# cheshmi/parsy_bench

Measured on AMD Instinct MI355X. Metric: Cholesky factorizations/sec (+ SpTRSV solves/sec), SuiteSparse SPD set, higher is better.
Workload: dtype f64; 1 GPU; flan-class stand-in (BASELINE.json configs[2] when flan: Flan_1565): grid (116, 116, 116) 27-point stencil, geometric nested dissection; n=1560896, nnz_A_lower=21491316, nsuper=81191, nnz_L=2044454227, xsize=2421483055, etree_levels=17, launches_per_factorization=357, parallelism=1 GPU

## Files before the change

### include/parsy_amd.h

```cpp
#ifndef PARSY_AMD_H
#define PARSY_AMD_H

#include <stdbool.h>
#include <stddef.h>
#include <stdint.h>

#ifdef __cplusplus
extern "C" {
#endif


bool cholesky_left_par_05(int n, int* c, int* r, double* values, size_t* lC, int* lR,
                          size_t* Li_ptr, double* lValues, int* blockSet, int supNo,
                          double* timing, int* aTree, int* cT, int* rT, int* col2Sup,
                          int nLevels, int* levelPtr, int* levelSet, int nPar, int* parPtr,
                          int* partition, int chunk, int threads, int super_max, int col_max,
                          double* nodCost);

bool cholesky_left_par_05_prune(int n, int* c, int* r, double* values, size_t* lC, int* lR,
                                size_t* Li_ptr, double* lValues, int* blockSet, int supNo,
                                double* timing, int* prunePtr, int* pruneSet, int nLevels,
                                int* levelPtr, int* levelSet, int nPar, int* parPtr, int* partition,
                                int chunk, int threads, int super_max, int col_max, double* nodCost);

// ... 52 lines not shown
    int32_t solve_one;
    int32_t solve_one_blocks;
    int32_t sub_mrhs_trees;
    int32_t sub_mrhs_slots;
    int32_t sub_mrhs_tiers;
    int32_t sub_mrhs_cover_level;
    int64_t dense_strip_entries;
} parsy_plan_info;

parsy_plan* parsy_plan_create(int n, int supNo, const int* blockSet, const size_t* lC,
                              const size_t* Li_ptr, const int* lR, const int* aTree,
                              const int* col2Sup, const int* cT, const int* rT, const int* c,
                              const int* r, int device);
void parsy_plan_destroy(parsy_plan* plan);
int parsy_plan_get_info(const parsy_plan* plan, parsy_plan_info* info);

int parsy_plan_set_active(parsy_plan* plan, const uint8_t* mask);
long long parsy_plan_chain_check(const parsy_plan* plan, int slots);
long long parsy_plan_check(const parsy_plan* plan);

int parsy_factor_device(parsy_plan* plan, const double* d_values, double* d_lValues,
                        void* stream);
#define PARSY_FACTOR_NO_INIT 1
int parsy_factor_device_ex(parsy_plan* plan, const double* d_values, double* d_lValues,
                           void* stream, int flags);
int parsy_factor_status(parsy_plan* plan);

int parsy_factor_begin(parsy_plan* plan, const double* d_values, double* d_lValues, void* stream, int flags);
int parsy_factor_level(parsy_plan* plan, int level, double* d_lValues, void* stream);
int parsy_factor_end(parsy_plan* plan, void* stream);
int parsy_plan_pieces(const parsy_plan* plan, int32_t* supernode, int32_t* level, int32_t* col0, int32_t* width,
                      int32_t* rows, int64_t* value_begin, int64_t* value_end);
int parsy_plan_set_active_pieces(parsy_plan* plan, const uint8_t* piece_mask);

typedef struct parsy_dist parsy_dist;
typedef struct parsy_dist_info {
    int32_t nranks, nlevels, n_pieces, n_subtrees, n_root_pieces, n_messages;
    int64_t exchange_elements;
    double total_cost, root_cost;
    double max_rank_cost;
    double lockstep_cost;
} parsy_dist_info;
parsy_dist* parsy_dist_create(const parsy_plan* plan, int nranks, int block);
void parsy_dist_destroy(parsy_dist* dist);
int parsy_dist_get_info(const parsy_dist* dist, parsy_dist_info* info);
int parsy_dist_get(const parsy_dist* dist, int32_t* owner, uint8_t* in_subtree, double* rank_cost,
                   double* level_cost);
int parsy_dist_level_messages(const parsy_dist* dist, int level);
int parsy_dist_message(const parsy_dist* dist, int level, int index, int32_t* src, int32_t* dst, int64_t* nseg,
                       int64_t* total, const int64_t** off, const int32_t** len, const int64_t** packed);
long long parsy_dist_check(const parsy_plan* plan, const parsy_dist* dist);

int parsy_solve_device(parsy_plan* plan, const double* d_lValues, double* d_x, int nrhs,
                       int ldx, void* stream);

int parsy_solve_status(parsy_plan* plan);

int parsy_backsolve_device(parsy_plan* plan, const double* d_lValues, double* d_x, int nrhs, int ldx,
                           void* stream);
int parsy_plan_solve_levels(const parsy_plan* plan, int32_t* level);
#define PARSY_SOLVE_FIRST 1
#define PARSY_SOLVE_LAST 2
#define PARSY_SOLVE_BACKWARD 4
int parsy_solve_levels_device(parsy_plan* plan, const double* d_lValues, double* d_x, int nrhs, int ldx, void* stream,
                              int level_begin, int level_end, int flags);
int parsy_rhs_ones_device(parsy_plan* plan, const double* d_lValues, double* d_b, void* stream);
// ... 163 lines not shown
```

### parsy_bench_amd/_native.py

```python
from __future__ import annotations

import ctypes as C
import os
from pathlib import Path

import numpy as np

_PKG = Path(__file__).resolve().parent
_LIB_PATH = Path(os.environ["PARSY_LIB"]) if os.environ.get("PARSY_LIB") else _PKG / "libparsy_amd.so"
_lib = None

c_int_p = C.POINTER(C.c_int)
c_dbl_p = C.POINTER(C.c_double)
c_size_p = C.POINTER(C.c_size_t)
c_i64_p = C.POINTER(C.c_int64)


class SymbolicView(C.Structure):
    _fields_ = [
        ("n", C.c_int32), ("nsuper", C.c_int32), ("nlevels", C.c_int32),
        ("maxSupWid", C.c_int32), ("maxCol", C.c_int32),
        ("ssize", C.c_int64), ("xsize", C.c_int64), ("nnzL", C.c_int64),
        ("nnzA", C.c_int64), ("n_updates", C.c_int64),
        ("flops_colcount", C.c_double), ("flops_stored", C.c_double),
# ... 29 lines not shown
        ("sub_mrhs_tiers", C.c_int32), ("sub_mrhs_cover_level", C.c_int32),
        ("dense_strip_entries", C.c_int64),
    ]

    def as_dict(self):
        return {k: getattr(self, k) for k, _ in self._fields_}


EXPORTED_SYMBOLS = [
    "cholesky_left_par_05", "cholesky_left_par_05_prune", "cholesky_left_par_waveFront", "blockedLsolve",
    "leveledBlockedLsolve", "H2LeveledBlockedLsolve", "H2LeveledBlockedLsolve_Peeled",
    "parsy_dropin_reset", "parsy_plan_create", "parsy_plan_destroy", "parsy_plan_get_info",
    "parsy_plan_set_active", "parsy_plan_chain_check", "parsy_factor_device", "parsy_factor_status", "parsy_solve_device",
    "parsy_factor_host", "parsy_solve_host", "parsy_last_factor_ms", "parsy_last_solve_ms",
    "parsy_last_error", "parsy_device_count", "parsy_analyze", "parsy_symbolic_free",
    "parsy_symbolic_get", "parsy_plan_from_symbolic", "parsy_grid_spd_lower",
    "parsy_grid_nested_dissection", "parsy_order_nd", "parsy_plan_profile", "parsy_plan_profile_collect",
    "parsy_plan_profile_get", "parsy_factor_device_ex", "parsy_backsolve_device", "parsy_solve_levels_device", "parsy_plan_solve_levels", "parsy_solve2_host",
    "parsy_rhs_ones_device", "parsy_solve_status", "parsy_copy_segments_device", "parsy_plan_check",
    "parsy_factor_begin", "parsy_factor_level", "parsy_factor_end", "parsy_plan_pieces",
    "parsy_plan_set_active_pieces", "parsy_dist_create", "parsy_dist_destroy", "parsy_dist_get_info",
    "parsy_dist_get", "parsy_dist_level_messages", "parsy_dist_message", "parsy_dist_check",
    "parsy_mg_create", "parsy_mg_destroy", "parsy_mg_set_values", "parsy_mg_factor", "parsy_mg_rank_ms",
    "parsy_mg_gather_host", "parsy_mg_dist", "parsy_mg_plan", "parsy_mg_profile", "parsy_plan_profile_levels",
    "parsy_debug_kernel_count", "parsy_debug_kernel_name", "parsy_debug_kernel_launches", "parsy_debug_kernel_reset",
    "parsy_plan_set_perm", "parsy_residual_device", "parsy_solve_spd_device", "parsy_solve_spd_host",
    "parsy_selinv_get_info", "parsy_selinv_check", "parsy_selinv_device", "parsy_inverse_diag_device",
    "parsy_selinv_host", "parsy_logdet_device",
    "parsy_plan_pattern", "parsy_grad_get_info", "parsy_pattern_outer_device", "parsy_inverse_pattern_device",
    "parsy_trace_inverse_device", "parsy_pattern_outer_host", "parsy_inverse_pattern_host",
    "parsy_cond_get_info", "parsy_error_bounds_device", "parsy_solve_spd_bounds_device", "parsy_solve_spd_bounds_host",
    "parsy_rcond_device", "parsy_rcond_host",
    "parsy_factor_apply_device", "parsy_factor_apply_host", "parsy_factor_apply_get_info", "parsy_factor_apply_row_index",
]


class ApplyInfo(C.Structure):
    _fields_ = [
        ("rows", C.c_int32), ("max_occurrences", C.c_int32), ("occurrences", C.c_int64), ("block_columns", C.c_int32),
        ("last_op", C.c_int32), ("last_launches", C.c_int32), ("reserved", C.c_int32), ("workspace_bytes", C.c_int64),
        ("device_bytes", C.c_int64),
    ]

    def as_dict(self):
        return {k: getattr(self, k) for k, _ in self._fields_ if k != "reserved"}


class CondInfo(C.Structure):
    _fields_ = [("applications", C.c_int32), ("columns", C.c_int32), ("device_bytes", C.c_int64)]

    def as_dict(self):
        return {k: getattr(self, k) for k, _ in self._fields_}


class GradInfo(C.Structure):
    _fields_ = [
        ("entries", C.c_int64), ("offdiag_entries", C.c_int64), ("device_bytes", C.c_int64), ("last_lanes", C.c_int32),
    ]

    def as_dict(self):
        return {k: getattr(self, k) for k, _ in self._fields_}


class SelinvInfo(C.Structure):
    _fields_ = [
        ("levels", C.c_int32), ("block_columns", C.c_int32), ("tiled_block_columns", C.c_int32),
# ... 31 lines not shown
    lib.parsy_symbolic_free.argtypes = [vp]
    lib.parsy_symbolic_get.argtypes = [vp, C.POINTER(SymbolicView)]
    lib.parsy_grid_spd_lower.restype = C.c_int64
    lib.parsy_grid_spd_lower.argtypes = [C.c_int, C.c_int, C.c_int, C.c_int, C.c_double, vp, vp, vp]
    lib.parsy_grid_nested_dissection.argtypes = [C.c_int, C.c_int, C.c_int, C.c_int, vp]
    lib.parsy_order_nd.argtypes = [C.c_int, vp, vp, C.c_int, vp]
    lib.parsy_plan_create.restype = vp
    lib.parsy_plan_create.argtypes = [C.c_int, C.c_int] + [vp] * 10 + [C.c_int]
    lib.parsy_plan_from_symbolic.restype = vp
    lib.parsy_plan_from_symbolic.argtypes = [vp, C.c_int]
    lib.parsy_plan_destroy.argtypes = [vp]
    lib.parsy_plan_get_info.argtypes = [vp, C.POINTER(PlanInfo)]
    lib.parsy_plan_set_active.argtypes = [vp, vp]
    lib.parsy_plan_chain_check.argtypes = [vp, C.c_int]
    lib.parsy_plan_chain_check.restype = C.c_longlong
    lib.parsy_plan_check.argtypes = [vp]
    lib.parsy_plan_check.restype = C.c_longlong
    lib.parsy_factor_device.argtypes = [vp, vp, vp, vp]
    lib.parsy_factor_device_ex.argtypes = [vp, vp, vp, vp, C.c_int]
    lib.parsy_factor_status.argtypes = [vp]
    lib.parsy_solve_device.argtypes = [vp, vp, vp, C.c_int, C.c_int, vp]
    lib.parsy_plan_solve_levels.argtypes = [vp, vp]
    lib.parsy_solve_levels_device.argtypes = [vp, vp, vp, C.c_int, C.c_int, vp, C.c_int, C.c_int, C.c_int]
    lib.parsy_backsolve_device.argtypes = [vp, vp, vp, C.c_int, C.c_int, vp]
    lib.parsy_solve2_host.argtypes = [vp, vp, vp, C.c_int, C.c_int, C.c_int, vp]
    lib.parsy_rhs_ones_device.argtypes = [vp, vp, vp, vp]
    lib.parsy_solve_status.argtypes = [vp]
    lib.parsy_copy_segments_device.argtypes = [vp, vp, vp, vp, vp, C.c_int64, vp]
    lib.parsy_factor_begin.argtypes = [vp, vp, vp, vp, C.c_int]
    lib.parsy_factor_level.argtypes = [vp, C.c_int, vp, vp]
    lib.parsy_factor_end.argtypes = [vp, vp]
    lib.parsy_plan_pieces.argtypes = [vp] + [vp] * 7
    lib.parsy_plan_set_active_pieces.argtypes = [vp, vp]
    lib.parsy_dist_create.restype = vp
    lib.parsy_dist_create.argtypes = [vp, C.c_int, C.c_int]
    lib.parsy_dist_destroy.argtypes = [vp]
    lib.parsy_dist_get_info.argtypes = [vp, C.POINTER(DistInfo)]
    lib.parsy_dist_get.argtypes = [vp, vp, vp, vp, vp]
    lib.parsy_dist_level_messages.argtypes = [vp, C.c_int]
    lib.parsy_dist_message.argtypes = [vp, C.c_int, C.c_int, c_int_p, c_int_p, c_i64_p, c_i64_p,
                                       C.POINTER(c_i64_p), C.POINTER(c_int_p), C.POINTER(c_i64_p)]
    lib.parsy_dist_check.argtypes = [vp, vp]
    lib.parsy_dist_check.restype = C.c_longlong
    lib.parsy_mg_create.restype = vp
    lib.parsy_mg_create.argtypes = [vp, C.c_int, vp, C.c_int]
    lib.parsy_mg_destroy.argtypes = [vp]
    lib.parsy_mg_set_values.argtypes = [vp, vp]
    lib.parsy_mg_factor.argtypes = [vp, vp]
    lib.parsy_mg_rank_ms.argtypes = [vp, vp]
    lib.parsy_mg_profile.argtypes = [vp, vp, vp, vp]
    lib.parsy_plan_profile_levels.argtypes = [vp, vp, vp]
    lib.parsy_mg_gather_host.argtypes = [vp, vp]
    lib.parsy_mg_dist.restype = vp
    lib.parsy_mg_dist.argtypes = [vp]
    lib.parsy_mg_plan.restype = vp
    lib.parsy_mg_plan.argtypes = [vp, C.c_int]
    lib.parsy_plan_set_perm.argtypes = [vp, vp]
    lib.parsy_residual_device.argtypes = [vp, vp, vp, C.c_int, vp, C.c_int, vp, C.c_int, C.c_int, vp, vp]
    lib.parsy_solve_spd_device.argtypes = [vp, vp, vp, vp, C.c_int, vp, C.c_int, C.c_int, C.c_int, vp, vp, vp]
    lib.parsy_solve_spd_host.argtypes = [vp, vp, vp, vp, C.c_int, vp, C.c_int, C.c_int, C.c_int, vp, vp, vp]
    lib.parsy_cond_get_info.argtypes = [vp, vp]
    lib.parsy_error_bounds_device.argtypes = [vp, vp, vp, vp, C.c_int, vp, C.c_int, C.c_int, vp, vp, vp]
    lib.parsy_solve_spd_bounds_device.argtypes = [vp, vp, vp, vp, C.c_int, vp, C.c_int, C.c_int, C.c_int, vp, vp, vp, vp]
    lib.parsy_solve_spd_bounds_host.argtypes = [vp, vp, vp, vp, C.c_int, vp, C.c_int, C.c_int, C.c_int, vp, vp, vp, vp]
    lib.parsy_rcond_device.argtypes = [vp, vp, vp, vp, vp, vp]
    lib.parsy_rcond_host.argtypes = [vp, vp, vp, vp, vp, vp]
# ... 83 lines not shown
```

### parsy_bench_amd/api.py

```python
from __future__ import annotations

import ctypes as C

import numpy as np

from . import _native as N

KIND_NAMES = ["SMALL", "TILES", "CHAIN", "BIG", "BACK_BELOW", "SOLVE_SMALL", "SOLVE_PANEL", "SOLVE_FIXUP", "BACK_BLOCK", "DENSE"]


def device_count() -> int:
    return int(N.lib().parsy_device_count())


def kernel_launches() -> dict:
    lib = N.lib()
    return {lib.parsy_debug_kernel_name(k).decode(): int(lib.parsy_debug_kernel_launches(k))
            for k in range(lib.parsy_debug_kernel_count())}


def reset_kernel_launches() -> None:
    N.lib().parsy_debug_kernel_reset()


# ... 433 lines not shown
            raise RuntimeError("parsy_solve_device failed: " + N.last_error())

    def solve_levels(self) -> np.ndarray:
        out = np.zeros(self.sym.nsuper, dtype=np.int32)
        N.lib().parsy_plan_solve_levels(self._h, N.ptr(out))
        return out

    def solve_levels_device(self, d_lValues: int, d_x: int, nrhs: int, ldx: int, stream: int, level_begin: int, level_end: int,
                            first: bool, last: bool, backward: bool = False) -> None:
        flags = (1 if first else 0) | (2 if last else 0) | (4 if backward else 0)
        if N.lib().parsy_solve_levels_device(self._h, d_lValues, d_x, nrhs, ldx, stream, level_begin, level_end, flags) != 0:
            raise RuntimeError("parsy_solve_levels_device failed: " + N.last_error())

    def factor_begin(self, d_values: int, d_lValues: int, stream: int = 0, init: bool = True) -> None:
        if N.lib().parsy_factor_begin(self._h, d_values, d_lValues, stream, 0 if init else 1) != 0:
            raise RuntimeError("parsy_factor_begin failed: " + N.last_error())

    def factor_level(self, level: int, d_lValues: int, stream: int = 0) -> None:
        if N.lib().parsy_factor_level(self._h, level, d_lValues, stream) != 0:
            raise RuntimeError("parsy_factor_level failed: " + N.last_error())

    def factor_end(self, stream: int = 0) -> None:
        if N.lib().parsy_factor_end(self._h, stream) != 0:
            raise RuntimeError("parsy_factor_end failed: " + N.last_error())

    def pieces(self) -> dict:
        n = int(N.lib().parsy_plan_pieces(self._h, *([None] * 7)))
        out = {k: np.zeros(n, dtype=np.int32) for k in ("supernode", "level", "col0", "width", "rows")}
        out.update({k: np.zeros(n, dtype=np.int64) for k in ("value_begin", "value_end")})
        N.lib().parsy_plan_pieces(self._h, *[N.ptr(out[k]) for k in (
            "supernode", "level", "col0", "width", "rows", "value_begin", "value_end")])
        return out

    def set_active_pieces(self, mask) -> None:
        m = None if mask is None else np.ascontiguousarray(mask, dtype=np.uint8)
        if N.lib().parsy_plan_set_active_pieces(self._h, N.ptr(m)) != 0:
            raise RuntimeError(N.last_error())

    def check(self) -> int:
        return int(N.lib().parsy_plan_check(self._h))

    def last_factor_ms(self) -> float:
        return float(N.lib().parsy_last_factor_ms(self._h))

    def last_solve_ms(self) -> float:
        return float(N.lib().parsy_last_solve_ms(self._h))

    def profile(self, mode: int) -> None:
        N.lib().parsy_plan_profile(self._h, mode)

    def profile_collect(self) -> None:
        if N.lib().parsy_plan_profile_collect(self._h) != 0:
            raise RuntimeError("profile_collect: no profiled run to collect")

    def profile_get(self) -> dict:
        ms = np.zeros(10, dtype=np.float64)
        cnt = np.zeros(10, dtype=np.int32)
        runs = C.c_int(0)
        N.lib().parsy_plan_profile_get(self._h, N.ptr(ms), N.ptr(cnt), C.byref(runs))
        return {"runs": runs.value, "ms": dict(zip(KIND_NAMES, ms.tolist())),
                "launches": dict(zip(KIND_NAMES, cnt.tolist()))}


class Dist:

    def __init__(self, plan: "Plan", nranks: int, block: int = 0, _borrowed=None):
# ... 106 lines not shown
```

### parsy_bench_amd/csrc/capi_exec.hip

```cpp
#include <hip/hip_runtime.h>

#include <chrono>
#include <cstdio>
#include <cstring>
#include <map>
#include <algorithm>
#include <mutex>
#include <string>
#include <tuple>
#include <vector>

#include "../../include/parsy_amd.h"
#include "errors.hpp"
#include "hip_check.hpp"
#include "dist.hpp"
#include "executor.hpp"
#include "inspector.hpp"
#include "plan_util.hpp"
#include "refine.hpp"
#include "cond.hpp"
#include "apply.hpp"

using parsy::set_last_error;

// ... 348 lines not shown
    parsy::build_launches(pl->S, mask, pl->piece_mask_set ? pieces.data() : nullptr);
    pl->sn_mask_set = mask != nullptr;
    return parsy::plan_upload_launches(pl);
}

int parsy_plan_set_active_pieces(parsy_plan* pl, const uint8_t* piece_mask) {
    if (!pl) return -1;
    std::vector<uint8_t> sn_mask;
    if (pl->sn_mask_set) sn_mask = pl->S.active;
    parsy::build_launches(pl->S, pl->sn_mask_set ? sn_mask.data() : nullptr, piece_mask);
    pl->piece_mask_set = piece_mask != nullptr;
    return parsy::plan_upload_launches(pl);
}

int parsy_plan_pieces(const parsy_plan* pl, int32_t* supernode, int32_t* level, int32_t* col0, int32_t* width,
                      int32_t* rows, int64_t* value_begin, int64_t* value_end) {
    if (!pl) return -1;
    const parsy::Schedule& S = pl->S;
    const int nc = (int)S.csn.size();
    for (int p = 0; p < nc; ++p) {
        const parsy::SnDesc& C = S.csn[(size_t)p];
        const parsy::SnDesc& R = S.sn[(size_t)S.csn_real[(size_t)p]];
        if (supernode) supernode[p] = S.csn_real[(size_t)p];
        if (level) level[p] = S.level_of.empty() ? 0 : S.level_of[(size_t)p];
        if (col0) col0[p] = C.c0;
        if (width) width[p] = C.w;
        if (rows) rows[p] = C.r;
        if (value_begin) value_begin[p] = R.px + (int64_t)C.rbias * R.r;
        if (value_end) value_end[p] = R.px + (int64_t)(C.rbias + C.w) * R.r;
    }
    return nc;
}

int parsy_plan_solve_levels(const parsy_plan* pl, int32_t* level) {
    if (!pl) return -1;
    const parsy::Schedule& S = pl->S;
    if (level)
        for (int l = 0; l < S.nlevels; ++l)
            for (int q = S.levelPtr[(size_t)l]; q < S.levelPtr[(size_t)l + 1]; ++q) level[S.levelSet[(size_t)q]] = l;
    return S.nlevels;
}

int64_t parsy_debug_big_entries(const parsy_plan* pl, int32_t* out, int64_t cap) {
    if (!pl) return -1;
    const parsy::Schedule& S = pl->S;
    int64_t n = 0, t = 0;
    for (const parsy::Schedule::BigTask& b : S.big_all) {
        for (int64_t e = b.e0; e < b.e1; ++e, ++n) {
            if (!out || n >= cap) continue;
            const parsy::WaveEntry& E = S.big_entries[(size_t)e];
            int32_t* o = out + 7 * n;
            o[0] = (int32_t)t;
            o[1] = b.src_level * 2 + (b.next ? 0 : 1);
            o[2] = E.K;
            o[3] = E.mn & 255;
            o[4] = (E.mn >> 8) & 255;
            o[5] = ((E.mn >> 16) & 1) != 0;
            o[6] = E.ia - E.ja;
        }
        ++t;
    }
    return n;
}

int64_t parsy_debug_big_windows(const parsy_plan* pl, int64_t* out, int64_t cap) {
    if (!pl) return -1;
// ... 398 lines not shown
```

### parsy_bench_amd/csrc/executor.hip

```cpp
#include "executor.hpp"

#include <climits>
#include <cstdlib>
#include <cstring>
#include <stdexcept>

#include "apply.hpp"
#include "cond.hpp"
#include "device_util.hpp"
#include "errors.hpp"
#include "grad.hpp"
#include "hip_check.hpp"
#include "plan_fwd.hpp"
#include "plan_util.hpp"
#include "refine.hpp"
#include "selinv.hpp"

namespace parsy {

const Schedule& plan_schedule(const parsy_plan* plan) { return plan->S; }

int check_plan(const parsy_plan* pl, const char* who, PlanNeeds needs) {
    const std::string w(who);
    if (pl->device < 0) return set_last_error(w + ": plan was built without a device (device < 0)"), -1;
// ... 202 lines not shown
        PARSY_HIP(hipMalloc(&d, sbytes));
        pl->owned.push_back(d);
        pl->dp.tile_scratch = (double*)d;
        pl->device_bytes += (int64_t)sbytes;
    }
    {
        void* d = nullptr;
        PARSY_HIP(hipMalloc(&d, sizeof(int)));
        pl->owned.push_back(d);
        pl->dp.info = (int*)d;
        PARSY_HIP(hipMemset(d, 0x7f, sizeof(int)));
        PARSY_HIP(hipMalloc(&d, sizeof(int)));
        pl->owned.push_back(d);
        pl->dp.sinfo = (int*)d;
        PARSY_HIP(hipMemset(d, 0, sizeof(int)));
        const size_t tbytes = 2 * std::max<int64_t>(S.n_tflags, 1) * sizeof(int);
        pl->dp.n_tflags = (int)S.n_tflags;
        PARSY_HIP(hipMalloc(&d, tbytes));
        pl->owned.push_back(d);
        pl->dp.tflags = (int*)d;
        PARSY_HIP(hipMemset(d, 0, tbytes));
        pl->device_bytes += (int64_t)tbytes;
    }
    {
        int prio_least = 0, prio_greatest = 0;
        PARSY_HIP(hipDeviceGetStreamPriorityRange(&prio_least, &prio_greatest));
        PARSY_HIP(hipStreamCreateWithPriority(&pl->side_stream, hipStreamNonBlocking, prio_least));
    }
    PARSY_HIP(hipEventCreateWithFlags(&pl->ev_init, hipEventDisableTiming));
    pl->ev_level_done.resize(std::max(S.nlevels, S.cnlevels) + 1);
    pl->ev_early_done.resize(std::max(S.nlevels, S.cnlevels) + 1);
    for (auto& e : pl->ev_level_done) PARSY_HIP(hipEventCreateWithFlags(&e, hipEventDisableTiming));
    for (auto& e : pl->ev_early_done) PARSY_HIP(hipEventCreateWithFlags(&e, hipEventDisableTiming));
    {
        const char* no = std::getenv("PARSY_NO_OVERLAP");
        pl->overlap = !(no && no[0] == '1');
    }
    PARSY_HIP(hipEventCreate(&pl->ev_f0));
    PARSY_HIP(hipEventCreate(&pl->ev_f1));
    PARSY_HIP(hipEventCreate(&pl->ev_s0));
    PARSY_HIP(hipEventCreate(&pl->ev_s1));
    return plan_upload_launches(pl);
}

parsy_plan* plan_build(const PatternRef& P, const size_t* lC, const int* A2p, const int* A2i,
                       int device) {
    parsy_plan* pl = new parsy_plan;
    int cus = 0;
    if (device >= 0) {
        hipDeviceProp_t prop;
        if (hipGetDeviceProperties(&prop, device) == hipSuccess) cus = prop.multiProcessorCount;
        (void)hipSetDevice(device);
        const int per_cu = chain_workgroups_per_cu();
        if (per_cu == 1) cus = cus / 2;
    }
    try {
        build_schedule(P, lC, A2p, A2i, nullptr, pl->S, cus);
    } catch (const std::exception& e) {
        set_last_error(std::string("plan: ") + e.what());
        delete pl;
        return nullptr;
    }
    pl->solve_only = pl->S.solve_only;
    pl->device = device;
    if (device >= 0 && plan_upload(pl) != 0) {
        plan_free(pl);
        return nullptr;
    }
    return pl;
}

void plan_free(parsy_plan* pl) {
    if (!pl) return;
    if (pl->device >= 0) {
        (void)hipSetDevice(pl->device);
        (void)hipDeviceSynchronize();
        for (void* d : pl->owned) (void)hipFree(d);
        for (void* d : pl->launch_owned) (void)hipFree(d);
        if (pl->xscratch) (void)hipFree(pl->xscratch);
        for (double*& q : pl->one_y) {
            if (q) (void)hipFree(q);
            q = nullptr;
        }
        if (pl->xt) (void)hipFree(pl->xt);
        if (pl->d_perm) (void)hipFree(pl->d_perm);
        if (pl->dinv) (void)hipFree(pl->dinv);
        if (pl->dp.bpart) (void)hipFree(pl->dp.bpart);
        if (pl->h_values_dev) (void)hipFree(pl->h_values_dev);
        if (pl->h_L_dev) (void)hipFree(pl->h_L_dev);
        if (pl->h_x_dev) (void)hipFree(pl->h_x_dev);
        for (hipEvent_t e : {pl->ev_f0, pl->ev_f1, pl->ev_s0, pl->ev_s1})
            if (e) (void)hipEventDestroy(e);
        for (hipEvent_t e : pl->pev) (void)hipEventDestroy(e);
        for (hipEvent_t e : pl->ev_level_done) (void)hipEventDestroy(e);
        for (hipEvent_t e : pl->ev_early_done) (void)hipEventDestroy(e);
        if (pl->ev_init) (void)hipEventDestroy(pl->ev_init);
        if (pl->side_stream) (void)hipStreamDestroy(pl->side_stream);
        if (pl->h_stream) (void)hipStreamDestroy(pl->h_stream);
        if (pl->h_copy) (void)hipStreamDestroy(pl->h_copy);
        for (hipEvent_t e : pl->h_band_ev) (void)hipEventDestroy(e);
    }
    refine_free(pl);
    selinv_free(pl);
    grad_free(pl);
    cond_free(pl);
    apply_free(pl);
    delete pl;
}

static void profile_mark(parsy_plan* pl, int kind, hipStream_t stream, size_t& cursor, int level = -1, int side = 0,
                         int count = 0) {
    if (!pl->profile) return;
    if (cursor >= pl->pev_count.size()) pl->pev_count.resize(cursor + 1, 0);
    pl->pev_count[cursor] = count;
    if (cursor >= pl->pev_level.size()) pl->pev_level.resize(cursor + 1, 0);
    pl->pev_level[cursor] = level >= 0 ? (level << 1) | (side & 1) : -1;
    if (cursor >= pl->pev.size()) {
        hipEvent_t e;
        (void)hipEventCreate(&e);
        pl->pev.push_back(e);
    }
    if (cursor >= pl->pev_kind.size()) pl->pev_kind.push_back(kind);
    else pl->pev_kind[cursor] = kind;
    (void)hipEventRecord(pl->pev[cursor], stream);
    ++cursor;
}

static bool sub_tiers_usable(const parsy_plan* pl, int nrhs, int ldx) {
    const int m = pl->dp.gates.sub_mrhs_min;
    return pl->dp.sub_ntiers > 0 && m > 0 && nrhs >= m && ldx < (1 << 24) && nrhs < (1 << 20);
}

static void run_begin(parsy_plan* pl) {
    pl->run_cursor = 0;
    pl->run_next_level_event = 0;
    pl->run_early_seen.assign(pl->ev_early_done.size(), 0);
}

static void run_range(parsy_plan* pl, const std::vector<Launch>& seq, size_t i0, size_t i1, double* L,
                      const double* Lc, double* x, int nrhs, int ldx, hipStream_t stream) {
    size_t& cursor = pl->run_cursor;
    const bool overlap = pl->overlap && !pl->profile && pl->side_stream != nullptr;
    int& next_level_event = pl->run_next_level_event;
    std::vector<char>& early_seen = pl->run_early_seen;
    auto record_levels_below = [&](int level) {
        for (; next_level_event < level && next_level_event < (int)pl->ev_level_done.size(); ++next_level_event)
            (void)hipEventRecord(pl->ev_level_done[next_level_event], stream);
    };
    for (size_t li = i0; li < i1; ++li) {
        const Launch& l = seq[li];
        const bool on_side = overlap && l.side;
        if (!on_side) {
            if (overlap && is_chol_launch(l.kind)) record_levels_below(l.level);
            if (overlap && (l.kind == kLaunchChain || l.kind == kLaunchBig || l.kind == kLaunchDense)) {
                int lw = std::min<int>(l.level, (int)early_seen.size() - 1);
                while (lw >= 0 && !early_seen[lw]) --lw;
                if (lw >= 0) (void)hipStreamWaitEvent(stream, pl->ev_early_done[lw], 0);
            }
        }
        profile_mark(pl, l.kind, stream, cursor, l.level, l.side, l.count);
        switch (l.kind) {
            case kLaunchSmall: launch_chol_small(pl->dp, l.first, l.count, l.lds_bytes, l.jb, l.fused == 2, L, stream); break;
            case kLaunchTiles:
            case kLaunchBig:
            case kLaunchDense: {
                const hipStream_t st = on_side ? pl->side_stream : stream;
                if (on_side) {
                    record_levels_below(l.wait_level + 1);
                    (void)hipStreamWaitEvent(st, l.wait_level >= 0 ? pl->ev_level_done[l.wait_level] : pl->ev_init, 0);
                }
                if (l.kind == kLaunchBig) launch_chol_big(pl->dp, l.first, l.count, L, st);
                else if (l.kind == kLaunchDense) launch_chol_dense(pl->dp, l.first, l.count, L, st);
                else launch_chol_tiles(pl->dp, l.first, l.count, L, st);
                if (on_side) {
                    (void)hipEventRecord(pl->ev_early_done[l.level], st);
                    early_seen[l.level] = 1;
                }
                break;
            }
            case kLaunchChain: launch_chol_chain(pl->dp, l.first, l.count, l.jb, pl->epoch, l.fused != 0, L, stream); break;
            case kLaunchSolveSmall:
                if (l.fused == 2 && sub_tiers_usable(pl, nrhs, ldx) && pl->S.sub_tiers[0].ntrees == l.count)
                    launch_solve_sub_mrhs(pl->dp, pl->S.sub_tiers[0], Lc, x, nrhs, ldx, pl->solve_ldq, stream);
                else
                    launch_solve_small(pl->dp, l.first, l.count, l.jb, l.fused == 2, Lc, x, nrhs, ldx, pl->solve_ldq, stream);
                break;
            case kLaunchSolvePanel:
                if (l.fused && nrhs >= pl->dp.gates.chain_mrhs_min)
                    launch_solve_blocks_mrhs(pl->dp, l.lds_bytes, l.wait_level, Lc, pl->dinv, x, pl->xscratch, nrhs, ldx,
                                             pl->solve_ldq, l.jb, pl->dp.gates.wait_bias, stream);
                else if (l.fused)
                    launch_solve_chain(pl->dp, l.first, l.count, Lc, pl->dinv, x, pl->xscratch, l.jb, pl->dp.gates.wait_bias,
                                       stream);
                else
                    launch_solve_panel(pl->dp, l.first, l.count, Lc, x, pl->xscratch, nrhs, ldx, stream);
                break;
            case kLaunchSolveFixup:
                launch_solve_fixup(pl->dp, l.first, l.count, x, pl->xscratch, nrhs, ldx, stream);
                break;
            case kLaunchBackBelow:
// ... 365 lines not shown
```

### parsy_bench_amd/csrc/executor.hpp

```cpp
#pragma once
#include <hip/hip_runtime.h>

#include <cstdint>
#include <mutex>
#include <string>
#include <vector>

#include "../../include/parsy_amd.h"
#include "kernels.hpp"
#include "schedule.hpp"

namespace parsy {
struct RefineState;
struct SelinvState;
struct GradState;
struct CondState;
struct ApplyState;
}

struct parsy_plan {
    parsy::Schedule S;
    int device = -1;
    std::mutex use_mu;
    bool solve_only = false;
    bool sn_mask_set = false, piece_mask_set = false;

    std::vector<void*> owned;
    std::vector<void*> launch_owned;
    parsy::DevicePattern dp;
    int64_t device_bytes = 0;
    int epoch = 0;

    double* dinv = nullptr;
    double* xscratch = nullptr;
    int64_t xscratch_len = 0;
    double* one_y[2] = {nullptr, nullptr};
    unsigned one_calls[2] = {0, 0};
    int one_cap[2] = {0, 0};
    int64_t one_bytes[2] = {0, 0};
    bool one_off = false, one_off_back = false;
    const int* solve_status_word = nullptr;

    double* h_values_dev = nullptr;
    double* h_L_dev = nullptr;
    double* h_x_dev = nullptr;
    int64_t h_values_len = 0, h_L_len = 0, h_x_len = 0;
    hipStream_t h_stream = nullptr, h_copy = nullptr;
    std::vector<hipEvent_t> h_band_ev;
    bool h_ready = false;
    bool levels_open = false, levels_backward = false;
    int levels_nrhs = 0;
    std::vector<int> h_band_level;
    std::vector<std::vector<std::pair<int64_t, int64_t>>> h_band_runs;

    hipStream_t side_stream = nullptr;
    hipEvent_t ev_init = nullptr;
    std::vector<hipEvent_t> ev_level_done, ev_early_done;
    bool overlap = true;

    size_t run_cursor = 0;
    int run_next_level_event = 0;
    std::vector<char> run_early_seen;
    bool factor_open = false;
    int factor_next_level = 0;

    hipEvent_t ev_f0 = nullptr, ev_f1 = nullptr, ev_s0 = nullptr, ev_s1 = nullptr;
    bool have_f = false, have_s = false;

    bool profile = false;
    double* xt = nullptr;
    int64_t xt_len = 0;
    int solve_ldq = 0;
    std::vector<hipEvent_t> pev;
    std::vector<int> pev_kind;
    std::vector<int> pev_level;
    std::vector<int> pev_count;
    std::vector<float> pev_ms;
    std::vector<double> level_ms;
    double kind_ms[PARSY_PROFILE_KINDS] = {};
    int kind_launches[PARSY_PROFILE_KINDS] = {};
    int profiled_runs = 0;
    std::vector<int> perm;
    int* d_perm = nullptr;
    parsy::RefineState* refine = nullptr;
    parsy::SelinvState* selinv = nullptr;
    parsy::GradState* grad = nullptr;
    parsy::CondState* cond = nullptr;
    parsy::ApplyState* apply = nullptr;
};

namespace parsy {

parsy_plan* plan_build(const PatternRef& P, const size_t* lC, const int* A2p, const int* A2i,
                       int device);
// ... 17 lines not shown
```

### parsy_bench_amd/csrc/schedule.cpp

```cpp
#include "schedule.hpp"

#include <cstdio>
#include <map>
#include <algorithm>
#include <queue>
#include <climits>
#include <cmath>
#include <cstdlib>
#include <cstdint>
#include <functional>
#include <stdexcept>
#include <string>

namespace parsy {

static inline int ceil_div(int a, int b) { return (a + b - 1) / b; }

static int env_int(const char* name, int dflt) {
    const char* v = std::getenv(name);
    if (!v || !*v) return dflt;
    return std::atoi(v);
}

static int find_subtrees(const std::vector<int>& parent, const std::vector<uint8_t>& eligible,
                         const std::vector<double>& cost, double cap, std::vector<int32_t>& subtree,
                         const std::vector<std::pair<int32_t, int32_t>>* slots = nullptr, int64_t slot_cap = 0) {
    const int ns = (int)parent.size();
    subtree.assign(ns, -1);
    std::vector<uint8_t> whole(eligible);
    std::vector<double> sub(cost);
    std::vector<int64_t> cols(slots ? ns : 0);
    for (int s = 0; s < ns && slots; ++s) cols[s] = (*slots)[s].first;
    for (int s = 0; s < ns; ++s) {
        const int p = parent[s];
        if (p < 0) continue;
        if (p <= s) return 0;
        if (!whole[s]) whole[p] = 0;
        sub[p] += sub[s];
        if (slots) cols[p] += cols[s];
    }
    int count = 0;
    for (int s = ns - 1; s >= 0; --s) {
        const int p = parent[s];
        if (p >= 0 && subtree[p] >= 0) subtree[s] = subtree[p];
        else if (whole[s] && sub[s] <= cap && (!slots || cols[s] + (*slots)[s].second <= slot_cap)) subtree[s] = count++;
    }
    return count;
}

void build_schedule(const PatternRef& P, const size_t* lC, const int* A2p, const int* A2i,
                    const uint8_t* active, Schedule& S, int compute_units) {
    S = Schedule();
    if (compute_units > 0) S.walker_batch = std::max(4, std::min(kWalkerBatch, compute_units / 2));
    const int n = P.n, ns = P.nsuper;
    S.n = n;
    S.nsuper = ns;
    S.solve_only = (A2p == nullptr);
    S.nnzA = A2p ? A2p[n] : 0;
    S.rows.assign(P.s, P.s + P.i_ptr[n]);
    S.ssize = (int64_t)P.i_ptr[n];
    S.xsize = (int64_t)lC[n];
    S.sn.resize(ns);
    for (int t = 0; t < ns; ++t) {
        SnDesc& d = S.sn[t];
        d.c0 = P.super[t];
        d.w = P.super[t + 1] - P.super[t];
        d.r = (int)(P.i_ptr[P.super[t + 1]] - P.i_ptr[P.super[t]]);
        d.ld = d.r;
        d.rbias = 0;
        d.px = (int64_t)lC[d.c0];
        d.pi = (int64_t)P.i_ptr[d.c0];
        d.a0 = A2p ? A2p[d.c0] : 0;
        d.a1 = A2p ? A2p[P.super[t + 1]] : 0;
        d.upd0 = 0;
        d.nupd = 0;
        d.dslot = -1;
        d.tflag0 = -1;
        if (d.w <= 0 || d.r < d.w) throw std::runtime_error("schedule: malformed supernode");
        if ((int64_t)d.w * d.r > 0x7fffffffLL)
            throw std::runtime_error("schedule: a single panel exceeds 2^31 entries");
        for (int col = d.c0; col < d.c0 + d.w; ++col)
            if (lC[col + 1] - lC[col] != (size_t)d.r || P.i_ptr[col] != P.i_ptr[d.c0])
                throw std::runtime_error("schedule: lC / Li_ptr are not a column-major panel layout");
        S.max_width = std::max(S.max_width, d.w);
        S.max_rows = std::max(S.max_rows, d.r);
        S.nnzL += (int64_t)d.w * d.r - (int64_t)d.w * (d.w - 1) / 2;
// ... 19 lines not shown
            const int row = S.rows[T.pi + k];
            map[row] = k;
            stamp[row] = t;
        }
        for (int col = T.c0; !S.solve_only && col < T.c0 + T.w; ++col)
            for (int q = A2p[col]; q < A2p[col + 1]; ++q) {
                const int row = A2i[q];
                if (stamp[row] != t) throw std::runtime_error("schedule: A entry outside the pattern of L");
                S.a_dst[q] = (int64_t)lC[col] + map[row];
            }
        for (int64_t u = uptr[t]; u < uptr[t + 1]; ++u) {
            const SnDesc& D = S.sn[usn[u]];
            urel[u] = (int64_t)S.relpos.size();
            for (int k = ulb[u]; k < D.r; ++k) {
                const int row = S.rows[D.pi + k];
                if (stamp[row] != t)
                    throw std::runtime_error("schedule: descendant row missing from the target's pattern");
                S.relpos.push_back(map[row]);
            }
            const double K = D.w, m = D.r - ulb[u], n1 = uub[u] - ulb[u] + 1;
            S.update_flops += K * n1 * (n1 + 1) + 2.0 * K * (m - n1) * n1;
            S.reread_bytes += 8.0 * K * m;
        }
    }
    if (S.relpos.size() > 0x7fffffffULL) throw std::runtime_error("schedule: relative index array exceeds int32");

    S.big_min_k = S.update_flops >= kBigAutoFlops ? kBigMinK : INT_MAX;
    S.piece_width = S.update_flops >= kPieceAutoFlops ? kPieceWidth : 0;
    if (std::getenv("PARSY_BIG_MINK")) S.big_min_k = std::max(1, env_int("PARSY_BIG_MINK", kBigMinK));
    if (std::getenv("PARSY_PIECE_WIDTH")) S.piece_width = env_int("PARSY_PIECE_WIDTH", kPieceWidth);
    if (S.piece_width > 0) S.piece_width = ceil_div(std::max(S.piece_width, kBigTile), kBigTile) * kBigTile;
    if (S.piece_width < S.big_min_k) S.piece_width = 0;
    S.push_group = std::max(1, env_int("PARSY_PUSH_GROUP", kPushGroup));
    const int split_chunks = env_int("PARSY_SPLIT_CHUNKS", kSplitChunks), split_target = std::max(1, env_int("PARSY_SPLIT_TARGET", kSplitTarget)),
              split_max = std::max(1, env_int("PARSY_SPLIT_MAX", kSplitMaxParts));
    const bool split_env = std::getenv("PARSY_SPLIT_CHUNKS") != nullptr;

    std::vector<int> tree(P.sparent, P.sparent + ns);
    S.sparent = tree;
    level_sets(tree, S.levelPtr, S.levelSet);
    S.nlevels = (int)S.levelPtr.size() - 1;

    S.piece0.assign(ns + 1, 0);
    for (int t = 0; t < ns; ++t) {
        const SnDesc& T = S.sn[t];
        S.piece0[t] = (int32_t)S.csn.size();
        int np = 1;
        const int pw = S.piece_width;
        if (!S.solve_only && pw > 0 && T.w > pw + pw / 2) {
            np = ceil_div(T.w, pw);
            if (T.w - (np - 1) * pw < pw / 2) --np;
        }
        for (int j = 0; j < np; ++j) {
            const int off = j * pw;
            SnDesc c = T;
            c.c0 = T.c0 + off;
            c.w = (j == np - 1) ? T.w - off : pw;
            c.r = T.r - off;
            c.ld = T.r;
            c.rbias = off;
            c.px = T.px + (int64_t)off * T.r + off;
            c.pi = T.pi + off;
            c.dslot = -1;
            S.csn.push_back(c);
            S.csn_real.push_back(t);
        }
// ... 904 lines not shown
                    const int nbc = ceil_div(T.w, kTile), nbr = ceil_div(T.r, kTile);
                    if (J >= nbc) continue;
                    auto push = [&](int I, int Jc) {
                        if (chain_split && ((I < nbc || !splits(t)) != (part == 0))) return;
                        const int64_t si = S.tile_split[S.sn_tw0[t] / 2 + (size_t)Jc * nbr + I];
                        S.tiles.push_back(TileDesc{t, I * kTile, Jc * kTile,
                                                   si < 0 ? 0 : S.split_desc[(size_t)si].nparts,
                                                   S.sn_wp0[t] + (((int64_t)Jc * nbr + I) * 2 + 1) * 4,
                                                   si < 0 ? -1 : S.split_desc[(size_t)si].sp});
                    };
                    if (J == 0) push(0, 0);
                    const bool next_diag = J + 1 < nbc;
                    if (next_diag) {
                        push(J + 1, J);
                        push(J + 1, J + 1);
                    }
                    for (int I = next_diag ? J + 2 : J + 1; I < nbr; ++I) push(I, J);
                }
            }
            Lc.count = (int32_t)S.tiles.size() - Lc.first;
            if (Lc.count > 0) S.chol.push_back(Lc);
            else --S.n_chain_launches;
            }
        }
    }
    S.chol_level_begin.assign(level_begin.begin(), level_begin.end());
    if (!early_launches.empty()) {
        std::vector<Launch> merged;
        size_t e = 0;
        std::stable_sort(early_launches.begin(), early_launches.end(),
                         [](const Launch& a, const Launch& b) { return a.level < b.level; });
        for (int lev = 0; lev < S.cnlevels; ++lev) {
            S.chol_level_begin[(size_t)lev] = merged.size();
            while (e < early_launches.size() && early_launches[e].level - 1 <= lev) merged.push_back(early_launches[e++]);
            const size_t b0 = level_begin[lev], b1 = lev + 1 < S.cnlevels ? level_begin[lev + 1] : S.chol.size();
            merged.insert(merged.end(), S.chol.begin() + b0, S.chol.begin() + b1);
        }
        S.chol.swap(merged);
    }
    S.chol_level_begin.push_back(S.chol.size());
    for (int lev = 0; lev < S.nlevels; ++lev) {
        sbigs.clear();
        if (lev == 0 && S.n_solve_subtrees > 0) {
            Launch L{kLaunchSolveSmall, 0, 0, 0, 0, 0, 2, 0, -1, 0};
            L.count = subtree_ranges(
                S.solve_subtree, S.n_solve_subtrees, S.solve_cost, [&] { return (int32_t)S.solve_small_list.size(); },
                [&](int32_t t) {
                    S.solve_small_list.push_back(t);
                    L.jb = std::max<int32_t>(L.jb, S.sn[t].w);
                },
                S.solve_small_ranges);
            if (L.count > 0) S.solve.push_back(L);
        }
        {
            std::vector<int32_t> tiny, narrow;
            for (int q = S.levelPtr[lev]; q < S.levelPtr[lev + 1]; ++q) {
                const int t = S.levelSet[q];
                if (!S.active[t] || S.solve_subtree[t] >= 0) continue;
                if (S.sn[t].w <= kTinyWidth) tiny.push_back(t);
                else if (S.sn[t].w <= kTile) narrow.push_back(t);
                else sbigs.push_back(t);
            }
            if (!narrow.empty() && tiny.size() < 64) {
                narrow.insert(narrow.end(), tiny.begin(), tiny.end());
                tiny.clear();
            }
            for (const std::vector<int32_t>* group : {&tiny, &narrow}) {
                if (group->empty()) continue;
                Launch L{kLaunchSolveSmall, (int32_t)S.solve_small_list.size(), (int32_t)group->size(), lev, 0, 0, 0, 0, -1, 0};
// ... 857 lines not shown
        for (const Launch& l : S.chol) {
            if (l.kind != kLaunchSmall) continue;
            if (l.fused == 2) {
                for (int b = l.first; b < l.first + l.count; ++b) {
                    const int32_t q0 = S.small_ranges[2 * (size_t)b], q1 = S.small_ranges[2 * (size_t)b + 1];
                    if (q0 < 0 || q1 <= q0 || q1 > (int32_t)S.small_list.size()) {
                        fail("subtree launch: bad range " + std::to_string(b));
                        continue;
                    }
                    for (int32_t q = q0; q < q1; ++q) {
                        seen[S.small_list[q]]++;
                        if (q > q0 && S.small_list[q] <= S.small_list[q - 1]) fail("subtree launch: a run is not in index order");
                        if (S.chol_subtree[S.csn_real[S.small_list[q]]] != S.chol_subtree[S.csn_real[S.small_list[q0]]])
                            fail("subtree launch: a run mixes subtrees");
                    }
                }
            } else {
                for (int q = l.first; q < l.first + l.count; ++q) seen[S.small_list[q]]++;
            }
        }
        for (int t = 0; t < nc; ++t)
            if (seen[t] != ((is_small(S.csn[t]) && S.active_piece[t]) ? 1 : 0))
                fail("SMALL supernode " + std::to_string(t) + " is in " + std::to_string(seen[t]) + " launches");
    }
    int main_level = -1;
    for (size_t i = 0; i < S.chol.size(); ++i) {
        const Launch& l = S.chol[i];
        if (l.side) {
            if (l.wait_level >= 0 && main_level > l.wait_level + 0 && main_level >= l.level)
                fail("side launch " + std::to_string(i) + " is enqueued after the level that waits for it");
            for (size_t j = i + 1; j < S.chol.size(); ++j)
                if (!S.chol[j].side && S.chol[j].level <= l.wait_level)
                    fail("side launch " + std::to_string(i) + " precedes a main-stream launch of a level it waits for");
        } else {
            if (l.level < main_level) fail("main-stream launches go down a level");
            main_level = l.level;
        }
    }
    return bad;
}

}
```

### parsy_bench_amd/csrc/schedule.hpp

```cpp
#pragma once
#include <cstddef>
#include <cstdint>
#include <string>
#include <vector>

#include "inspector.hpp"

namespace parsy {

constexpr int kTile = 64;
constexpr int kSub = 32;
constexpr int kSmallMaxEntries = 6144;
constexpr int kSmallMaxWidth = 64;
constexpr int kBelowRows = 512;
constexpr int kBelowMaxGroups = 512;
constexpr int kBackGroup = 2;
constexpr int kTinyWidth = 16;
constexpr int kTinyWidth2 = 32;
constexpr int kPanelRows = 128;
constexpr int kSolveRows = 256;
constexpr int kSolveRowsMrhs = 128;

struct SnDesc {
    int64_t px;
// ... 83 lines not shown
    int32_t first, count;
    int32_t level;
    int32_t jb;
    int32_t lds_bytes;
    int32_t fused;
    int32_t side;
    int32_t wait_level;
    int32_t early;
};

constexpr int kSplitChunks = 192;
constexpr int kSplitTarget = 128;
constexpr int kSplitMaxParts = 4;
constexpr int kSplitFewTiles = 128;
constexpr int kSplitFewChunks = 32;
constexpr int kSplitFewTarget = 24;
constexpr int kSplitFewMaxParts = 8;
constexpr int kWalkerBatch = 64;
constexpr int kBigTile = 128;
constexpr int kBigMinK = 128;
constexpr int kPieceWidth = 512;
constexpr double kBigAutoFlops = 1e11;
constexpr double kPieceAutoFlops = 2e12;
constexpr double kChainSplitAutoFlops = 1e11;
constexpr int kBigSuperMinTasks = 12288;
constexpr double kBigSuperMaxFill = 0.85;
constexpr int kBigGroup = 8;
constexpr int kBigGroupsPerXcd = 2;
constexpr int kBigTailGroups = 16;
constexpr int kDenseChunk = 8;
constexpr double kDenseMinShare = 0.25;
constexpr double kDenseMinFill = 0.70;
constexpr double kDenseAllShare = 0.06;
constexpr int kPushGroup = 1;
constexpr int kOneMaxSupernodes = 8192;
constexpr int64_t kOneLargeEntries = 4096;
constexpr int64_t kOneMaxEntries = 1 << 28;
constexpr int kOneMaxSupernodesBig = 32768;
constexpr int kOneSmallBlocks = 1024;
constexpr int kOneMidBlocks = 4096;
constexpr int kOneRhs8Density = 300;
constexpr int kOneMaxRhs = 8;
constexpr int kCholSubtreesPerCu = 64;
constexpr int kSubtreesPerCu = 16;
constexpr double kSubtreeMinCost = 2e5;
constexpr int kSubtreeMinPerSlot = 2;
constexpr int kSolveSubtreeMinMembers = 2048;

struct Schedule {
    int n = 0, nsuper = 0, nlevels = 0;
    bool solve_only = false;
    int64_t nnzA = 0, ssize = 0, xsize = 0, nnzL = 0;
    int max_width = 0, max_rows = 0, n_small = 0, n_big = 0;
    int n_solve_wide = 0;
    int64_t n_dslots = 0;
    int64_t n_tflags = 0;
    int n_chain_launches = 0;
    int n_solve_chain_launches = 0;
    int walker_batch = kWalkerBatch;
    double flops_stored = 0, update_flops = 0, reread_bytes = 0;
    double tile_update_flops = 0;
    double inner_flops = 0;

    std::vector<SnDesc> sn;
    std::vector<int> sparent;
    std::vector<SnDesc> csn;
    std::vector<int32_t> piece0;
    std::vector<int32_t> csn_real;
    std::vector<int> clevelPtr, clevelSet;
    int cnlevels = 0;
    int big_min_k = kBigMinK, piece_width = kPieceWidth, push_group = kPushGroup;
    int big_super_r = 0, big_super_c = 0;
    std::vector<UpdDesc> upd;
    std::vector<int32_t> upd_src;
    std::vector<int32_t> relpos;
    std::vector<int64_t> a_dst;
    std::vector<int32_t> rows;
    std::vector<WaveEntry> wave_entries;
    std::vector<int64_t> wave_ptr;

    std::vector<int32_t> chol_subtree, solve_subtree, bsolve_subtree;
    std::vector<int32_t> solve_subtree_all, bsolve_subtree_all;
    std::vector<double> chol_cost, solve_cost;
    int n_chol_subtrees = 0, n_solve_subtrees = 0, n_bsolve_subtrees = 0;
    std::vector<int32_t> small_ranges, solve_small_ranges, bsolve_ranges;
    std::vector<SubMember> sub_members;
    std::vector<SubTree> sub_trees;
    std::vector<uint16_t> sub_slots;
    std::vector<int32_t> sub_out_rows;
    std::vector<SubTier> sub_tiers;
    int sub_cover_level = -1;
    int sub_max_slots = 0;

    std::vector<int32_t> small_list;
    std::vector<TileDesc> tiles;
    std::vector<WaveEntry> big_entries;
    struct BigTask { int32_t sn, row0, col0, weight; int64_t e0, e1; int32_t src_level, next;
                     int32_t sr, sc;
                     int64_t em; int32_t dweight, dchunks;
                     int32_t strips; };
    std::vector<BigTask> big_all;
    std::vector<TileDesc> big_tasks;
    double big_flops = 0;
    double dense_flops = 0;
// ... 60 lines not shown
```

Measured before the change: 2.984 factorizations/s.

## Issue side-stream PUSH updates right after a level's NEXT big launches

Reorders the merged Cholesky launch list so that side-stream PUSH big/dense updates from a source level are placed right after the main stream's NEXT big launches of the following level. They wait on a new per-level event recorded at that point, instead of waiting for the whole source level to finish. A cost-model gate (task weights, compute-unit count, a chain-hop constant) decides per level whether to use this ordering, so the critical-path NEXT work gets the GPU first while PUSH work overlaps the rest. It also adds a schedule check and an API that exports the chol launch list. The risk is extra events and waits, plus a heuristic that may delay PUSH work when it misjudges.

Result: no change. 2.989 factorizations/s, median of 6 (+0.2%).

```diff
diff --git a/include/parsy_amd.h b/include/parsy_amd.h
--- a/include/parsy_amd.h
+++ b/include/parsy_amd.h
@@ -108,6 +108,7 @@
 int parsy_plan_pieces(const parsy_plan* plan, int32_t* supernode, int32_t* level, int32_t* col0, int32_t* width,
                       int32_t* rows, int64_t* value_begin, int64_t* value_end);
 int parsy_plan_set_active_pieces(parsy_plan* plan, const uint8_t* piece_mask);
+int parsy_plan_chol_launches(const parsy_plan* plan, int32_t* out);
 
 typedef struct parsy_dist parsy_dist;
 typedef struct parsy_dist_info {
diff --git a/parsy_bench_amd/_native.py b/parsy_bench_amd/_native.py
--- a/parsy_bench_amd/_native.py
+++ b/parsy_bench_amd/_native.py
@@ -85,6 +85,7 @@
     "parsy_cond_get_info", "parsy_error_bounds_device", "parsy_solve_spd_bounds_device", "parsy_solve_spd_bounds_host",
     "parsy_rcond_device", "parsy_rcond_host",
     "parsy_factor_apply_device", "parsy_factor_apply_host", "parsy_factor_apply_get_info", "parsy_factor_apply_row_index",
+    "parsy_plan_chol_launches",
 ]
 
 
@@ -182,6 +183,7 @@
     lib.parsy_factor_end.argtypes = [vp, vp]
     lib.parsy_plan_pieces.argtypes = [vp] + [vp] * 7
     lib.parsy_plan_set_active_pieces.argtypes = [vp, vp]
+    lib.parsy_plan_chol_launches.argtypes = [vp, vp]
     lib.parsy_dist_create.restype = vp
     lib.parsy_dist_create.argtypes = [vp, C.c_int, C.c_int]
     lib.parsy_dist_destroy.argtypes = [vp]
diff --git a/parsy_bench_amd/api.py b/parsy_bench_amd/api.py
--- a/parsy_bench_amd/api.py
+++ b/parsy_bench_amd/api.py
@@ -489,6 +489,13 @@
             "supernode", "level", "col0", "width", "rows", "value_begin", "value_end")])
         return out
 
+    def chol_launches(self) -> dict:
+        n = int(N.lib().parsy_plan_chol_launches(self._h, None))
+        out = np.zeros((n, 8), dtype=np.int32)
+        N.lib().parsy_plan_chol_launches(self._h, N.ptr(out))
+        return {k: out[:, q].copy() for q, k in enumerate(
+            ("kind", "level", "side", "wait_level", "early", "count", "first", "step"))}
+
     def set_active_pieces(self, mask) -> None:
         m = None if mask is None else np.ascontiguousarray(mask, dtype=np.uint8)
         if N.lib().parsy_plan_set_active_pieces(self._h, N.ptr(m)) != 0:
diff --git a/parsy_bench_amd/csrc/capi_exec.hip b/parsy_bench_amd/csrc/capi_exec.hip
--- a/parsy_bench_amd/csrc/capi_exec.hip
+++ b/parsy_bench_amd/csrc/capi_exec.hip
@@ -404,6 +404,20 @@
     return nc;
 }
 
+int parsy_plan_chol_launches(const parsy_plan* pl, int32_t* out) {
+    if (!pl) return -1;
+    const parsy::Schedule& S = pl->S;
+    size_t step = 0;
+    for (size_t i = 0; out && i < S.chol.size(); ++i) {
+        while (step + 1 < S.chol_level_begin.size() && S.chol_level_begin[step + 1] <= i) ++step;
+        const parsy::Launch& l = S.chol[i];
+        const int32_t row[8] = {l.kind, l.level, l.side, l.side ? l.wait_level : -1, l.side ? l.early : 0, l.count, l.first,
+                                (int32_t)step};
+        std::memcpy(out + 8 * i, row, sizeof(row));
+    }
+    return (int)S.chol.size();
+}
+
 int parsy_plan_solve_levels(const parsy_plan* pl, int32_t* level) {
     if (!pl) return -1;
     const parsy::Schedule& S = pl->S;
diff --git a/parsy_bench_amd/csrc/executor.hip b/parsy_bench_amd/csrc/executor.hip
--- a/parsy_bench_amd/csrc/executor.hip
+++ b/parsy_bench_amd/csrc/executor.hip
@@ -258,6 +258,8 @@
     pl->ev_early_done.resize(std::max(S.nlevels, S.cnlevels) + 1);
     for (auto& e : pl->ev_level_done) PARSY_HIP(hipEventCreateWithFlags(&e, hipEventDisableTiming));
     for (auto& e : pl->ev_early_done) PARSY_HIP(hipEventCreateWithFlags(&e, hipEventDisableTiming));
+    pl->ev_next_done.resize(pl->ev_level_done.size());
+    for (auto& e : pl->ev_next_done) PARSY_HIP(hipEventCreateWithFlags(&e, hipEventDisableTiming));
     {
         const char* no = std::getenv("PARSY_NO_OVERLAP");
         pl->overlap = !(no && no[0] == '1');
@@ -320,6 +322,7 @@
         for (hipEvent_t e : pl->pev) (void)hipEventDestroy(e);
         for (hipEvent_t e : pl->ev_level_done) (void)hipEventDestroy(e);
         for (hipEvent_t e : pl->ev_early_done) (void)hipEventDestroy(e);
+        for (hipEvent_t e : pl->ev_next_done) (void)hipEventDestroy(e);
         if (pl->ev_init) (void)hipEventDestroy(pl->ev_init);
         if (pl->side_stream) (void)hipStreamDestroy(pl->side_stream);
         if (pl->h_stream) (void)hipStreamDestroy(pl->h_stream);
@@ -360,6 +363,7 @@
 static void run_begin(parsy_plan* pl) {
     pl->run_cursor = 0;
     pl->run_next_level_event = 0;
+    pl->run_next_done_level = -1;
     pl->run_early_seen.assign(pl->ev_early_done.size(), 0);
 }
 
@@ -391,7 +395,13 @@
             case kLaunchBig:
             case kLaunchDense: {
                 const hipStream_t st = on_side ? pl->side_stream : stream;
-                if (on_side) {
+                if (on_side && l.early == 2) {
+                    if (pl->run_next_done_level != l.wait_level) {
+                        (void)hipEventRecord(pl->ev_next_done[l.wait_level], stream);
+                        pl->run_next_done_level = l.wait_level;
+                    }
+                    (void)hipStreamWaitEvent(st, pl->ev_next_done[l.wait_level], 0);
+                } else if (on_side) {
                     record_levels_below(l.wait_level + 1);
                     (void)hipStreamWaitEvent(st, l.wait_level >= 0 ? pl->ev_level_done[l.wait_level] : pl->ev_init, 0);
                 }
diff --git a/parsy_bench_amd/csrc/executor.hpp b/parsy_bench_amd/csrc/executor.hpp
--- a/parsy_bench_amd/csrc/executor.hpp
+++ b/parsy_bench_amd/csrc/executor.hpp
@@ -56,10 +56,12 @@
     hipStream_t side_stream = nullptr;
     hipEvent_t ev_init = nullptr;
     std::vector<hipEvent_t> ev_level_done, ev_early_done;
+    std::vector<hipEvent_t> ev_next_done;
     bool overlap = true;
 
     size_t run_cursor = 0;
     int run_next_level_event = 0;
+    int run_next_done_level = -1;
     std::vector<char> run_early_seen;
     bool factor_open = false;
     int factor_next_level = 0;
diff --git a/parsy_bench_amd/csrc/schedule.cpp b/parsy_bench_amd/csrc/schedule.cpp
--- a/parsy_bench_amd/csrc/schedule.cpp
+++ b/parsy_bench_amd/csrc/schedule.cpp
@@ -52,6 +52,7 @@
                     const uint8_t* active, Schedule& S, int compute_units) {
     S = Schedule();
     if (compute_units > 0) S.walker_batch = std::max(4, std::min(kWalkerBatch, compute_units / 2));
+    S.compute_units = compute_units > 0 ? compute_units : 256;
     const int n = P.n, ns = P.nsuper;
     S.n = n;
     S.nsuper = ns;
@@ -137,6 +138,8 @@
     if (S.piece_width > 0) S.piece_width = ceil_div(std::max(S.piece_width, kBigTile), kBigTile) * kBigTile;
     if (S.piece_width < S.big_min_k) S.piece_width = 0;
     S.push_group = std::max(1, env_int("PARSY_PUSH_GROUP", kPushGroup));
+    S.push_after_next = std::max(0, std::min(2, env_int("PARSY_PUSH_AFTER_NEXT", 1)));
+    S.push_gate = std::max(0, env_int("PARSY_PUSH_GATE", kPushGatePercent)) / 100.0;
     const int split_chunks = env_int("PARSY_SPLIT_CHUNKS", kSplitChunks), split_target = std::max(1, env_int("PARSY_SPLIT_TARGET", kSplitTarget)),
               split_max = std::max(1, env_int("PARSY_SPLIT_MAX", kSplitMaxParts));
     const bool split_env = std::getenv("PARSY_SPLIT_CHUNKS") != nullptr;
@@ -1107,9 +1110,45 @@
                          [](const Launch& a, const Launch& b) { return a.level < b.level; });
         for (int lev = 0; lev < S.cnlevels; ++lev) {
             S.chol_level_begin[(size_t)lev] = merged.size();
-            while (e < early_launches.size() && early_launches[e].level - 1 <= lev) merged.push_back(early_launches[e++]);
+            const size_t e0 = e;
+            while (e < early_launches.size() && early_launches[e].level - 1 <= lev) ++e;
             const size_t b0 = level_begin[lev], b1 = lev + 1 < S.cnlevels ? level_begin[lev + 1] : S.chol.size();
-            merged.insert(merged.end(), S.chol.begin() + b0, S.chol.begin() + b1);
+            auto is_big = [](const Launch& l) { return l.kind == kLaunchBig || l.kind == kLaunchDense; };
+            size_t next_end = b0;
+            for (size_t q = b0; q < b1; ++q)
+                if (is_big(S.chol[q])) next_end = q + 1;
+            size_t em = e;
+            bool behind = S.push_after_next == 2;
+            if (S.push_after_next == 1 && next_end > b0) {
+                auto alone = [&](const std::vector<const Schedule::BigTask*>& tasks) {
+                    int64_t sum = 0, top = 0;
+                    for (const Schedule::BigTask* b : tasks) {
+                        sum += (int64_t)b->weight + b->dweight;
+                        top = std::max<int64_t>(top, (int64_t)b->weight + b->dweight);
+                    }
+                    return std::max<double>((double)top, (double)sum / (2.0 * S.compute_units));
+                };
+                int nbc = 0;
+                for (int q = S.clevelPtr[lev]; q < S.clevelPtr[lev + 1]; ++q) {
+                    const int t = S.clevelSet[q];
+                    if (S.active_piece[t] && !is_small(S.csn[t]) && S.chol_subtree[S.csn_real[t]] < 0)
+                        nbc = std::max(nbc, ceil_div(S.csn[t].w, kTile));
+                }
+                behind = alone(big_push[lev - 1]) <= S.push_gate * (alone(big_next[lev - 1]) + (double)nbc * kChainHopUnits);
+            }
+            if (behind && next_end > b0)
+                for (size_t q = e0; q < e; ++q)
+                    if (is_big(early_launches[q]) && early_launches[q].wait_level == lev - 1) {
+                        em = q;
+                        break;
+                    }
+            if (em == e) next_end = b0;
+            for (size_t q = em; q < e; ++q)
+                if (is_big(early_launches[q])) early_launches[q].early = 2;
+            merged.insert(merged.end(), early_launches.begin() + e0, early_launches.begin() + em);
+            merged.insert(merged.end(), S.chol.begin() + b0, S.chol.begin() + next_end);
+            merged.insert(merged.end(), early_launches.begin() + em, early_launches.begin() + e);
+            merged.insert(merged.end(), S.chol.begin() + next_end, S.chol.begin() + b1);
         }
         S.chol.swap(merged);
     }
@@ -2033,6 +2072,24 @@
             for (size_t j = i + 1; j < S.chol.size(); ++j)
                 if (!S.chol[j].side && S.chol[j].level <= l.wait_level)
                     fail("side launch " + std::to_string(i) + " precedes a main-stream launch of a level it waits for");
+            if (l.kind == kLaunchBig || l.kind == kLaunchDense) {
+                auto is_next = [&](const Launch& m) {
+                    return !m.side && (m.kind == kLaunchBig || m.kind == kLaunchDense) && m.level == l.wait_level + 1;
+                };
+                size_t before = 0, after = 0;
+                for (size_t j = 0; j < S.chol.size(); ++j)
+                    if (is_next(S.chol[j])) ++(j < i ? before : after);
+                if (l.early == 2) {
+                    size_t j = i;
+                    while (j > 0 && S.chol[j - 1].side) --j;
+                    if (after > 0 || j == 0 || !is_next(S.chol[j - 1]))
+                        fail("PUSH launch " + std::to_string(i) + " is not right behind the NEXT launches of its source level");
+                } else if (before > 0 || (S.push_after_next == 2 && after > 0)) {
+                    fail("PUSH launch " + std::to_string(i) + " is not where its wait says (NEXT launches of its source level)");
+                }
+            } else if (l.early == 2) {
+                fail("side launch " + std::to_string(i) + " waits for NEXT launches but is no PUSH");
+            }
         } else {
             if (l.level < main_level) fail("main-stream launches go down a level");
             main_level = l.level;
diff --git a/parsy_bench_amd/csrc/schedule.hpp b/parsy_bench_amd/csrc/schedule.hpp
--- a/parsy_bench_amd/csrc/schedule.hpp
+++ b/parsy_bench_amd/csrc/schedule.hpp
@@ -139,6 +139,8 @@
 constexpr double kDenseMinShare = 0.25;
 constexpr double kDenseMinFill = 0.70;
 constexpr double kDenseAllShare = 0.06;
+constexpr int kChainHopUnits = 14;
+constexpr int kPushGatePercent = 60;
 constexpr int kPushGroup = 1;
 constexpr int kOneMaxSupernodes = 8192;
 constexpr int64_t kOneLargeEntries = 4096;
@@ -177,6 +179,9 @@
     std::vector<int> clevelPtr, clevelSet;
     int cnlevels = 0;
     int big_min_k = kBigMinK, piece_width = kPieceWidth, push_group = kPushGroup;
+    int push_after_next = 1;
+    double push_gate = kPushGatePercent / 100.0;
+    int compute_units = 256;
     int big_super_r = 0, big_super_c = 0;
     std::vector<UpdDesc> upd;
     std::vector<int32_t> upd_src;
```
